# horizon-research/Fov-3DGS

Measured on AMD Instinct MI355X. Metric: frames/sec at 1080p foveated (bicycle-scale), higher is better.
Workload: dtype f32; 1 GPU; S-6M bicycle-scale cloud, 4-layer foveated render (fov_pcheck_obb), the reference's 9 fixed gazes (0.25 i, 0.25 j) in turn, one camera per GPU; gaussians=6000000, width=1920, height=1080, sh_degree=3, model_layout=the reference's tensor interface (render(packed=None)), overlap_successive_frames=True, parallelism=views1

## Files before the change

fov-3dgs_amd/csrc/api.hip:

```cpp
#include "common.h"
#include <atomic>
#include <mutex>
#include <cstdarg>
#include <cstdio>
#include <cstring>
#include <cstdlib>
#include <new>

namespace fr {

static thread_local char g_err[512] = "";

void set_error(const char *fmt, ...)
{
	va_list ap;
	va_start(ap, fmt);
	vsnprintf(g_err, sizeof(g_err), fmt, ap);
	va_end(ap);
}

int check_launch(const char *what, hipStream_t stream, bool debug)
{
	hipError_t e = hipGetLastError();
	static const bool trace = getenv("FR_TRACE") != nullptr;
// ... 3 lines not shown
	if (e != hipSuccess)
	{
		set_error("%s: %s", what, hipGetErrorString(e));
		return FR_ERR_HIP;
	}
	return FR_OK;
}

#define FR_HIP(call) do { hipError_t e_ = (call); if (e_ != hipSuccess) { set_error("%s: %s", #call, hipGetErrorString(e_)); return FR_ERR_HIP; } } while (0)

static int validate_forward(const fr_forward_args *a)
{
	if (!a) { set_error("null args"); return FR_ERR_INVALID; }
	if (a->variant < FR_VARIANT_ORIGINAL || a->variant > FR_VARIANT_MMFR_PCHECK_OBB) { set_error("unknown variant %d", a->variant); return FR_ERR_INVALID; }
	if (a->P < 0 || a->W <= 0 || a->H <= 0) { set_error("bad sizes P=%d W=%d H=%d", a->P, a->W, a->H); return FR_ERR_INVALID; }
	if (a->P > (1 << 30) || a->W > 16 * 65535 || a->H > 16 * 65535) { set_error("too large: P=%d (max 2^30) W=%d H=%d (max 65535 tiles per axis)", a->P, a->W, a->H); return FR_ERR_INVALID; }
	if ((int64_t)((a->W + FR_TILE - 1) / FR_TILE) * ((a->H + FR_TILE - 1) / FR_TILE) >= (1 << 29)) { set_error("too many tiles (W=%d H=%d)", a->W, a->H); return FR_ERR_INVALID; }
	if (!a->out_color) { set_error("out_color is null"); return FR_ERR_INVALID; }
	if (a->P == 0) return FR_OK;
	if (!a->means3D || !a->opacities || !a->viewmatrix || !a->projmatrix || !a->campos || !a->background || !a->radii)
	{ set_error("a required pointer is null"); return FR_ERR_INVALID; }
	if (!a->geometry_resize || !a->binning_resize || !a->image_resize) { set_error("resize callbacks are required"); return FR_ERR_INVALID; }
	const bool fov = a->variant == FR_VARIANT_FOV_PCHECK_OBB;
	if (fov)
	{
		if (a->shs_rest) { set_error("shs_rest is not used by the foveated variant (its shs already is the rest part)"); return FR_ERR_INVALID; }
		if (!a->shs || !a->shs_dcs || !a->highest_levels) { set_error("foveated variant needs shs (rest), shs_dcs and highest_levels"); return FR_ERR_INVALID; }
		if (a->M != 15) { set_error("foveated variant expects M=15 rest coefficients, got %d", a->M); return FR_ERR_INVALID; }
	}
	else if (a->variant == FR_VARIANT_NAIVE_FOV_PCHECK_OBB || a->variant == FR_VARIANT_MMFR_PCHECK_OBB)
	{
// ... 554 lines not shown
```

fov-3dgs_amd/csrc/common.h:

```cpp
#pragma once
#include <hip/hip_runtime.h>
#include <stdint.h>
#include <stddef.h>
#include "../../include/fovraster.h"

#define FR_TILE 16
#define FR_TILE_PIX 256
#define FR_FOV_LEVELS 4
#define FR_SORT_LDS_MAX 8192
#ifndef FR_BIN_THREADS
#define FR_BIN_THREADS 768
#endif
#define FR_BIN_BLOCKS 512
#define FR_PROJ_MAX_WAVES 8192
#define FR_CROW_PAD (64 * FR_PROJ_MAX_WAVES)
#define FR_LDS_HIST_MAX_TILES 16384
#define FR_ITEM_NONE 0xffffffffu
#define FR_LDS_HIST16_MAX_TILES 34816
#define FR_HIST16_MAX_SLABS (65535 / FR_BIN_THREADS)
#define FR_BIG_TNUM 64
#define FR_GIANT_TNUM 1024
#define FR_GIANT_MAX 64
#define FR_SORT_SPLIT_MIN 16384
#define FR_SORT_CHUNK_TARGET 960
// ... 12 lines not shown
__host__ __device__ inline size_t align_up(size_t x, size_t a = 256) { return (x + a - 1) / a * a; }

struct GeomWS {
	float4 *rec;
	float *cov3D;
	float4 *acc;
	float4 *wrec;
	float4 *lvl;
	uint32_t *lrange;
	uint32_t *slab_ctr;
	uint32_t *vis_list;
	uint32_t *vis_seg;
	uint32_t *proj_counts;
	uint32_t *wbase;
	float4 *crow;
	size_t bytes;
};
__host__ __device__ inline GeomWS carve_geom(int variant, size_t P, char *base)
{
	GeomWS g; size_t off = 0;
	g.rec = (float4 *)(base + off); off = align_up(off + P * 3 * sizeof(float4));
	const bool keeps = has_backward(variant);
	g.cov3D = (float *)(base + off); off = align_up(off + P * (keeps ? 16 : 6) * sizeof(float));
	g.acc = nullptr;
	if (keeps) { g.acc = (float4 *)(base + off); off = align_up(off + P * 4 * sizeof(float4)); }
	g.lvl = nullptr;
	g.wrec = (float4 *)(base + off); off = align_up(off + P * 4 * sizeof(float4));
	if (variant == FR_VARIANT_FOV_PCHECK_OBB) { g.lvl = (float4 *)(base + off); off = align_up(off + P * FR_FOV_LEVELS * sizeof(float4)); }
	g.lrange = (uint32_t *)(base + off); off = align_up(off + P * sizeof(uint32_t));
	g.slab_ctr = (uint32_t *)(base + off); off = align_up(off + FR_SLAB_CTR_WORDS * sizeof(uint32_t));
	g.vis_list = (uint32_t *)(base + off); off = align_up(off + P * sizeof(uint32_t));
	g.vis_seg = (uint32_t *)(base + off); off = align_up(off + (P + FR_CROW_PAD) * sizeof(uint32_t));
	g.proj_counts = (uint32_t *)(base + off); off = align_up(off + FR_PROJ_MAX_WAVES * sizeof(uint32_t));
	g.wbase = (uint32_t *)(base + off); off = align_up(off + (FR_PROJ_MAX_WAVES + 1) * sizeof(uint32_t));
	g.crow = nullptr;
	if (is_fov(variant)) { g.crow = (float4 *)(base + off); off = align_up(off + (P + FR_CROW_PAD) * 3 * sizeof(float4)); }
	g.bytes = off + 256;
	return g;
}

struct ImageWS {
	float *final_T;
	uint32_t *n_contrib;
	uint2 *ranges;
	uint32_t *tile_count;
	uint32_t *lv_bbox;
	uint32_t *totals;
	uint32_t *render_items;
	uint32_t *tile_order;
	float *tile_lv;
	uint32_t *hist;
// ... 299 lines not shown
```

fov-3dgs_amd/csrc/preprocess.hip:

```cpp
#include "common.h"
#include "tile_scan.h"
#include <cstdlib>

namespace fr {

struct M3 { float c[3][3]; };
__device__ __forceinline__ M3 m3_cols(float a0, float a1, float a2, float b0, float b1, float b2, float c0, float c1, float c2)
{
	M3 m; m.c[0][0] = a0; m.c[0][1] = a1; m.c[0][2] = a2; m.c[1][0] = b0; m.c[1][1] = b1; m.c[1][2] = b2;
	m.c[2][0] = c0; m.c[2][1] = c1; m.c[2][2] = c2; return m;
}
__device__ __forceinline__ M3 m3_mul(const M3 &a, const M3 &b)
{
	M3 r;
#pragma unroll
	for (int col = 0; col < 3; col++)
#pragma unroll
		for (int row = 0; row < 3; row++)
			r.c[col][row] = a.c[0][row] * b.c[col][0] + a.c[1][row] * b.c[col][1] + a.c[2][row] * b.c[col][2];
	return r;
}
__device__ __forceinline__ M3 m3_t(const M3 &a)
{
	M3 r;
// ... 996 lines not shown
			}
			else
			{
				gidx = (int)a.geom.vis_seg[slot];
				load_candidate<PACKED, FOV>(a, gidx, g);
			}
		}
		GeomOut go;
		geom_item<VARIANT>(a, cam_vm, cam_pm, s_lvbox, valid, gidx, g, !PACKED && !FOV && a.raw && a.cov3D_precomp == nullptr, go);
		if (valid)
		{
			a.radii[gidx] = go.alive ? go.radius : 0;
			if (a.visibility) a.visibility[gidx] = (go.alive && go.radius > 0) ? 1 : 0;
			a.geom.vis_list[item] = (uint32_t)gidx;
		}
		rows_store<4>(go.wrow, orec, a.geom.wrec + 4 * (size_t)slab * 64, nv, lane);
		rows_store<3>(go.rrow, orec, a.geom.rec + 3 * (size_t)slab * 64, nv, lane);
		if (a.write_cov3D)
		{
			rows_store<4>(go.stash, orec, (float4 *)a.geom.cov3D + 4 * (size_t)slab * 64, nv, lane);
			const float4 ac[4] = { make_float4(0.f, 0.f, 0.f, 0.f), make_float4(0.f, 0.f, 0.f, 0.f), make_float4(0.f, 0.f, 0.f, 0.f), make_float4(go.inv_qnorm, 0.f, 0.f, 0.f) };
			rows_store<4>(ac, orec, a.geom.acc + 4 * (size_t)slab * 64, nv, lane);
		}
#pragma unroll
		for (int i = 0; i < 4; i++) wr[i] = go.wrow[i];
		fpos = make_float3(go.rrow[1].z, go.rrow[1].w, go.rrow[2].x);
		fconic = make_float3(go.rrow[0].z, go.rrow[0].w, go.rrow[1].x);
	}
	const uint32_t idf = __float_as_uint(wr[2].x), xy = __float_as_uint(wr[2].z);
	const int idx = (int)(idf & 0x3fffffffu);
	const bool alive = item < V && ((idf >> 30) & 1u) != 0, boxtest = ((idf >> 31) & 1u) != 0;
	const float4 ev = make_float4(wr[0].z, wr[0].w, wr[1].x, wr[1].y);
	const float2 el = make_float2(wr[1].z, wr[1].w);
	const int x0 = (int)(xy & 0xffffu), y0 = (int)(xy >> 16), ow0 = (int)__float_as_uint(wr[2].w);
	const uint32_t tnum = alive ? __float_as_uint(wr[3].x) : 0u;
	const float hl = wr[3].y;
	uint32_t count = 0;
	float lowest = hl, highest = 0;
	bool be_blend = false;
	const bool in_place = alive && tnum == 1 && !boxtest;
	if (in_place)
	{
		bool keep = true;
		const int ti = y0 * a.gx + x0;
		if (FOV)
		{
			uint32_t lb;
			TILE_FILTER(ti, hl + 1, keep, lb);
			if (keep) { const float level = (float)(31 - __clz((int)(lb & 15u))); lowest = level; highest = level; be_blend = (lb & 16u) != 0u; }
		}
		if (keep) { BUMP_TILE(ti); count = 1; }
	}
	bool deferred = false;
	{
		uint32_t lvmask = 0;
		if (alive && !in_place && tnum >= FR_GIANT_TNUM)
		{
			const uint32_t slot = atomicAdd(&s_ng, 1u);
			if (slot < FR_GIANT_MAX) { s_gitem[slot] = item; deferred = true; }
		}
		const bool big = alive && !in_place && !deferred && tnum >= FR_BIG_TNUM;
		if (__ballot(big)) __builtin_amdgcn_s_setprio(3);
		for (unsigned long long bigm = __ballot(big); bigm; bigm &= bigm - 1)
		{
			const int L = __ffsll((long long)bigm) - 1;
			const int ox0 = bcast_i(x0, L), oy0 = bcast_i(y0, L), ow = bcast_i(ow0, L);
// ... 54 lines not shown
					const bool cx_ok = !((o2.y - tpx) < -8.0f || (o2.x - tpx) > 8.0f);
					const bool cy_ok = !((o2.w - tpy) < -8.0f || (o2.z - tpy) > 8.0f);
					const float xp = tpx + 8.0f - o0.x, xm = tpx - 8.0f - o0.x, yp = tpy + 8.0f - o0.y, ym = tpy - 8.0f - o0.y;
					const float a1p = xp * o0.z, a1m = xm * o0.z, b1p = yp * o0.w, b1m = ym * o0.w;
					const float mn1 = fminf(a1p, a1m) + fminf(b1p, b1m), mx1 = fmaxf(a1p, a1m) + fmaxf(b1p, b1m);
					const bool e1_ok = !(o1.z < mn1 || -o1.z > mx1);
					const float a2p = xp * o1.x, a2m = xm * o1.x, b2p = yp * o1.y, b2m = ym * o1.y;
					const float mn2 = fminf(a2p, a2m) + fminf(b2p, b2m), mx2 = fmaxf(a2p, a2m) + fmaxf(b2p, b2m);
					const bool e2_ok = !(o1.w < mn2 || -o1.w > mx2);
					pass = pass && cx_ok && cy_ok && e1_ok && e2_ok;
				}
				if (FOV) m = pass ? lb : 0u;
			}
			if (pass) BUMP_TILE(ti);
			const unsigned long long mine = seg_mask(seg_a, seg_b);
			count += (uint32_t)__popcll(__ballot(pass) & mine);
			if (FOV)
			{
#pragma unroll
				for (int bit = 0; bit < 5; bit++)
					if (__ballot((m >> bit) & 1u) & mine) lvmask |= 1u << bit;
			}
		}
		if (total != 0)
		{
			__builtin_amdgcn_fence(__ATOMIC_RELEASE, "wavefront");
			__builtin_amdgcn_wave_barrier();
		}
		if (FOV && (my_n != 0 || big) && count != 0) range_from_mask(lvmask, lowest, highest, be_blend);
	}
	const uint32_t lr = (alive && !deferred) ? range_word(count, lowest, highest, be_blend) : FR_ITEM_NONE;
	if (item < V && !deferred) a.geom.lrange[item] = lr;
	if (alive && !deferred && count == 0) { a.radii[idx] = 0; if (a.visibility) a.visibility[idx] = 0; }
	if (__any(lr != FR_ITEM_NONE))
	{
		float4 r[3], lv[FR_FOV_LEVELS];
		r[0] = make_float4(wr[0].x, wr[0].y, fconic.x, fconic.y);
		r[1] = make_float4(fconic.z, LEVELCOL ? hl : 0.0f, fpos.x, fpos.y);
		r[2] = make_float4(fpos.z, wr[2].y, (FOV && !LEVELCOL) ? hl : 0.0f, __int_as_float(idx));
#pragma unroll
		for (int l = 0; l < FR_FOV_LEVELS; l++) lv[l] = make_float4(0, 0, 0, 0);
		if (lr != FR_ITEM_NONE) colour_item<VARIANT, PACKED>(a, rows_ok, lr, r, lv);
		if (LEVELCOL) rows_store<4>(lv, orec, a.geom.lvl + 4 * (size_t)slab * 64, nv, lane);
		else rows_store<3>(r, orec, a.geom.rec + 3 * (size_t)slab * 64, nv, lane);
	}
	}
	__syncthreads();
// ... 11 lines not shown
	}
	__syncthreads();
	if ((int)threadIdx.x < ng)
	{
		const int gitem = s_gitem[threadIdx.x];
		const uint32_t gcount = s_gcount[threadIdx.x];
		const float4 w2 = a.geom.wrec[4 * (size_t)gitem + 2], w3 = a.geom.wrec[4 * (size_t)gitem + 3];
		float lowest = w3.y, highest = 0.0f;
		bool be_blend = false;
		if (FOV && gcount != 0) range_from_mask(s_gmask[threadIdx.x], lowest, highest, be_blend);
		const uint32_t lr = range_word(gcount, lowest, highest, be_blend);
		a.geom.lrange[gitem] = lr;
		if (gcount == 0)
		{
			const uint32_t gi = __float_as_uint(w2.x) & 0x3fffffffu;
			a.radii[gi] = 0;
			if (a.visibility) a.visibility[gi] = 0;
		}
		else
		{
			float4 r[3], lv[FR_FOV_LEVELS];
#pragma unroll
			for (int i = 0; i < 3; i++) r[i] = a.geom.rec[3 * (size_t)gitem + i];
#pragma unroll
			for (int l = 0; l < FR_FOV_LEVELS; l++) lv[l] = make_float4(0, 0, 0, 0);
			colour_item<VARIANT, PACKED>(a, rows_ok, lr, r, lv);
			if (LEVELCOL)
			{
#pragma unroll
				for (int l = 0; l < FR_FOV_LEVELS; l++) a.geom.lvl[(size_t)gitem * FR_FOV_LEVELS + l] = lv[l];
// ... 29 lines not shown
			tile_scan_body<FR_TILE_SCAN_THREADS, true>(a.ts, lds_hist);
		}
	}
}
#undef BUMP_TILE
#undef TILE_FILTER

struct EmitArgs {
	int P, gx, gy, T;
	const int *radii;
	GeomWS geom;
	const float *highest_levels;
	const float *tile_lv;
	const uint32_t *lv_bbox;
	int lds_tiles;
	const uint2 *ranges;
	uint32_t *cursor;
	uint64_t *entries;
	const uint32_t *hist;
	const uint32_t *totals;
	uint32_t capacity;
	uint32_t items_cap;
};
#ifndef FR_EMIT_THREADS
#define FR_EMIT_THREADS FR_BIN_THREADS
#endif
#define NEXT_SLOT(ti) (LDSH == 2 ? a.ranges[(ti)].x + pre_row[(ti)] + ((atomicAdd(&lds_cur[(ti) >> 1], 1u << (16 * ((ti) & 1))) >> (16 * ((ti) & 1))) & 0xffffu) \
	: LDSH ? atomicAdd(&lds_cur[(ti)], 1u) : a.ranges[(ti)].x + atomicAdd(&a.cursor[(ti)], 1u))
template <int VARIANT, int LDSH>
__global__ void __launch_bounds__(FR_EMIT_THREADS) k_emit(const EmitArgs a)
{
	constexpr bool CULL = VARIANT != FR_VARIANT_ORIGINAL;
	constexpr bool FOV = VARIANT == FR_VARIANT_FOV_PCHECK_OBB;
	extern __shared__ __attribute__((aligned(16))) uint32_t lds_cur[];
#ifdef FR_EMIT_TIMERS
	const uint64_t tm_entry = wall_clock64(); uint64_t tm_pro = 0, tm_loop = 0, tm_walk = 0, tm_big = 0, tm_drain = 0, tm_pre = 0, tm_mid = 0, tm_ta = 0; int tm_slabs = 0, tm_steps = 0;
#endif
	if (a.totals[0] > a.capacity || a.totals[5] > a.items_cap) return;
	const int lane = threadIdx.x & 63;
	const int cur_words = LDSH == 2 ? (a.T + 1) / 2 : (LDSH ? a.T : 0);
	const uint32_t *const pre_row = a.hist + (LDSH ? (size_t)blockIdx.x * a.T : 0);
	uint32_t *lds_tab = lds_cur + cur_words;
	const int tab_words = (a.T + 7) / 8;
	const bool ldst = FOV && a.lds_tiles && a.geom.slab_ctr[3] == 0u;
	if (ldst)
	{
		const float *gmin = a.tile_lv + a.T;
		for (int t0 = threadIdx.x; t0 < a.T; t0 += 16 * FR_EMIT_THREADS)
		{
			float v[16];
#pragma unroll
// ... 12 lines not shown
#define TILE_PASSES(ti, olim) (ldst ? (float)((lds_tab[(ti) >> 3] >> (4 * ((ti) & 7))) & 7u) < (olim) : tile_min[(ti)] < (olim))
	if (LDSH == 2)
		for (int t = threadIdx.x; t < cur_words; t += FR_EMIT_THREADS) lds_cur[t] = 0;
	else if (LDSH)
	{
		const uint32_t *pre = pre_row;
		for (int t0 = threadIdx.x; t0 < a.T; t0 += 16 * FR_EMIT_THREADS)
		{
			uint32_t st[16], pr[16];
#pragma unroll
			for (int k = 0; k < 16; k++) { const int t = min(t0 + k * FR_EMIT_THREADS, a.T - 1); st[k] = a.ranges[t].x; pr[k] = pre[t]; }
#pragma unroll
			for (int k = 0; k < 16; k++) if (t0 + k * FR_EMIT_THREADS < a.T) lds_cur[t0 + k * FR_EMIT_THREADS] = st[k] + pr[k];
		}
	}
	__syncthreads();
	__shared__ int s_own[FR_EMIT_THREADS];
	float4 *const s_orec = (float4 *)(lds_cur + ((cur_words + (ldst ? tab_words : 0) + 3) & ~3));
	__shared__ int s_gidx[FR_GIANT_MAX];
	__shared__ uint32_t s_ng, s_next_slab;
	if (threadIdx.x == 0) { s_ng = 0; s_next_slab = 0; }
	__syncthreads();
#ifdef FR_EMIT_TIMERS
	tm_pro = wall_clock64() - tm_entry;
#endif
	const float *tile_min = FOV ? a.tile_lv + a.T : nullptr;
	auto walk_uniform = [&](const int ox0, const int oy0, const int ow, const uint32_t on, const Obb &ob, const float olim,
		const uint64_t opay, const uint32_t k0, const uint32_t kstep) __attribute__((always_inline))
	{
		const float rw = 1.0f / (float)ow;
		for (uint32_t k = k0; k < on; k += kstep)
		{
			const uint32_t j = k + lane;
			const bool valid = j < on;
			int ry = (int)(((float)j + 0.5f) * rw);
			int rx = (int)j - ry * ow;
			if (rx < 0) { ry--; rx += ow; } else if (rx >= ow) { ry++; rx -= ow; }
			const int x = ox0 + rx, y = oy0 + ry;
			const int ti = valid ? y * a.gx + x : 0;
			bool pass = valid;
			if (CULL)
			{
				if (FOV) pass = pass && TILE_PASSES(ti, olim);
				pass = pass && obb_hits_tile(ob, x, y);
			}
			if (pass) a.entries[NEXT_SLOT(ti)] = opay;
		}
	};
	const int V = (int)a.geom.slab_ctr[1];
	const int nslabs = (V + 63) / 64;
	struct SlabIn { float4 w0, w1, w2, w3; uint32_t lr; };
	auto fetch_slab = [&](const int slab, SlabIn &in) __attribute__((always_inline))
	{
		const int item = min(slab * 64 + lane, max(V - 1, 0));
		const float4 *wr = a.geom.wrec + 4 * (size_t)item;
		in.lr = a.geom.lrange[item];
		in.w0 = wr[0]; in.w1 = wr[1]; in.w2 = wr[2]; in.w3 = wr[3];
	};
	auto process = [&](const int slab, const SlabIn &in) __attribute__((always_inline))
	{
	const int item = slab * 64 + lane;
	int idx = 0;
	bool alive = false, boxtest = false;
	int x0 = 0, y0 = 0, x1 = 0;
	uint32_t tnum = 0;
	float cx = 0.f, cy = 0.f, hl = 0.f;
	uint32_t depth_bits = 0;
	float4 ev = make_float4(0, 0, 0, 0);
	float2 el = make_float2(0, 0);
	if (item < V)
	{
		const uint32_t lr = in.lr;
		const float4 w0 = in.w0, w1 = in.w1, w2 = in.w2, w3 = in.w3;
		const uint32_t idf = __float_as_uint(w2.x), xy = __float_as_uint(w2.z);
		idx = (int)(idf & 0x3fffffffu);
		alive = lr != FR_ITEM_NONE && ((idf >> 30) & 1u) != 0; boxtest = (idf >> 31) & 1u;
		cx = w0.x; cy = w0.y; ev = make_float4(w0.z, w0.w, w1.x, w1.y); el = make_float2(w1.z, w1.w);
		depth_bits = __float_as_uint(w2.y);
		x0 = (int)(xy & 0xffffu); y0 = (int)(xy >> 16); x1 = x0 + (int)__float_as_uint(w2.w);
		tnum = alive ? __float_as_uint(w3.x) : 0u;
		hl = w3.y;
	}
	const uint64_t payload = ((uint64_t)depth_bits << 32) | (uint32_t)item;
	const bool in_place = alive && tnum == 1 && !boxtest;
	if (in_place) a.entries[NEXT_SLOT(y0 * a.gx + x0)] = payload;
	{
		bool deferred = false;
		if (alive && !in_place && tnum >= FR_GIANT_TNUM)
		{
			const uint32_t slot = atomicAdd(&s_ng, 1u);
			if (slot < FR_GIANT_MAX) { s_gidx[slot] = item; deferred = true; }
		}
		const bool big = alive && !in_place && !deferred && tnum >= FR_BIG_TNUM;
#ifdef FR_EMIT_TIMERS
		const uint64_t tg0 = wall_clock64(); tm_pre += tg0 - tm_ta;
#endif
		for (unsigned long long bigm = __ballot(big); bigm; bigm &= bigm - 1)
		{
			const int L = __ffsll((long long)bigm) - 1;
			const int ox0 = bcast_i(x0, L), oy0 = bcast_i(y0, L), ow = bcast_i(x1, L) - ox0;
			const float4 oev = make_float4(bcast_f(ev.x, L), bcast_f(ev.y, L), bcast_f(ev.z, L), bcast_f(ev.w, L));
			const float2 oel = make_float2(bcast_f(el.x, L), bcast_f(el.y, L));
			const Obb ob = make_obb(bcast_f(cx, L), bcast_f(cy, L), oev, oel);
			const uint64_t opay = ((uint64_t)(uint32_t)bcast_i((int)depth_bits, L) << 32) | (uint32_t)(slab * 64 + L);
			walk_uniform(ox0, oy0, ow, (uint32_t)bcast_i((int)tnum, L), ob, bcast_f(hl, L) + 1, opay, 0u, 64u);
		}
#ifdef FR_EMIT_TIMERS
		const uint64_t tg1 = wall_clock64(); tm_big += tg1 - tg0;
#endif
		const uint32_t my_n = (alive && !in_place && !big && !deferred) ? tnum : 0u;
		const uint32_t incl = wave_incl_scan_u32(my_n, lane);
		const uint32_t excl = incl - my_n;
		const uint32_t total = (uint32_t)__builtin_amdgcn_readlane((int)incl, 63);
		float4 *const orec = s_orec + 4 * (threadIdx.x & ~63);
#ifdef FR_EMIT_TIMERS
		const uint64_t tw0 = wall_clock64(); tm_steps += (int)((total + 63) / 64); tm_mid += tw0 - tg1;
#endif
		if (total != 0)
		{
			const Obb ob = make_obb(cx, cy, ev, el);
			float4 *mine = orec + 4 * lane;
			mine[0] = make_float4(cx, cy, ev.x, ev.y);
			mine[1] = make_float4(ev.z, ev.w, el.x, el.y);
			mine[2] = make_float4(ob.vxmin, ob.vxmax, ob.vymin, ob.vymax);
			mine[3] = make_float4(__uint_as_float((uint32_t)x0 | ((uint32_t)y0 << 16)), __int_as_float(max(x1 - x0, 1)), __uint_as_float(excl), hl + 1);
			FR_WAVE_LDS_SYNC();
		}
		for (uint32_t k = 0; k < total; k += 64)
		{
			const uint32_t j = k + lane;
			const bool valid = j < total;
			const int seg_a = (int)max((long long)excl - (long long)k, 0ll);
			const int seg_b = (int)min((long long)incl - (long long)k, 64ll);
			const int owner = max(pair_owner_scan(s_own + (threadIdx.x & ~63), lane, seg_a, seg_b), 0);
			const float4 *orow = orec + 4 * owner;
			const float4 o3 = orow[3];
			const uint32_t oxy = __float_as_uint(o3.x);
			const int ow = __float_as_int(o3.y);
			const uint32_t local = (valid ? j : total - 1) - __float_as_uint(o3.z);
			int qy = (int)(((float)local + 0.5f) * __builtin_amdgcn_rcpf((float)ow));
			int rx = (int)local - qy * ow;
			if (rx < 0) { qy--; rx += ow; } else if (rx >= ow) { qy++; rx -= ow; }
			const int x = (int)(oxy & 0xffffu) + rx, y = (int)(oxy >> 16) + qy;
			const int ti = y * a.gx + x;
			const uint64_t opay = ((uint64_t)(uint32_t)__shfl((int)depth_bits, owner) << 32) | (uint32_t)(slab * 64 + owner);
			bool pass = valid;
			if (CULL)
			{
				const float4 o0 = orow[0], o1 = orow[1], o2 = orow[2];
				if (FOV) pass = pass && TILE_PASSES(valid ? ti : 0, o3.w);
				{
					const float tpx = (float)x * (float)FR_TILE + (float)FR_TILE / 2.0f, tpy = (float)y * (float)FR_TILE + (float)FR_TILE / 2.0f;
					const bool cx_ok = !((o2.y - tpx) < -8.0f || (o2.x - tpx) > 8.0f);
					const bool cy_ok = !((o2.w - tpy) < -8.0f || (o2.z - tpy) > 8.0f);
					const float xp = tpx + 8.0f - o0.x, xm = tpx - 8.0f - o0.x, yp = tpy + 8.0f - o0.y, ym = tpy - 8.0f - o0.y;
					const float a1p = xp * o0.z, a1m = xm * o0.z, b1p = yp * o0.w, b1m = ym * o0.w;
					const float mn1 = fminf(a1p, a1m) + fminf(b1p, b1m), mx1 = fmaxf(a1p, a1m) + fmaxf(b1p, b1m);
					const bool e1_ok = !(o1.z < mn1 || -o1.z > mx1);
					const float a2p = xp * o1.x, a2m = xm * o1.x, b2p = yp * o1.y, b2m = ym * o1.y;
					const float mn2 = fminf(a2p, a2m) + fminf(b2p, b2m), mx2 = fmaxf(a2p, a2m) + fmaxf(b2p, b2m);
					const bool e2_ok = !(o1.w < mn2 || -o1.w > mx2);
					pass = pass && cx_ok && cy_ok && e1_ok && e2_ok;
				}
			}
			if (pass) a.entries[NEXT_SLOT(ti)] = opay;
		}
		if (total != 0)
		{
			__builtin_amdgcn_fence(__ATOMIC_RELEASE, "wavefront");
			__builtin_amdgcn_wave_barrier();
		}
#ifdef FR_EMIT_TIMERS
		tm_walk += wall_clock64() - tw0;
#endif
	}
	};
	{
		constexpr int BW = FR_BIN_THREADS / 64;
		const int bin_waves = (int)gridDim.x * BW;
		auto slab_of = [&](const int s) { return (int)blockIdx.x * BW + s % BW + (s / BW) * bin_waves; };
		auto grab = [&]() -> int {
			uint32_t q_ = 0;
			if (lane == 0) q_ = atomicAdd(&s_next_slab, 1u);
			return slab_of(__builtin_amdgcn_readfirstlane((int)q_));
		};
		SlabIn cur, nxt;
		int slab = grab();
		if (slab < nslabs) fetch_slab(slab, cur);
#ifdef FR_EMIT_TIMERS
		const uint64_t tl0 = wall_clock64();
#endif
		for (; slab < nslabs; )
		{
#ifdef FR_EMIT_TIMERS
			tm_ta = wall_clock64();
#endif
			const int next = grab();
			const bool more = next < nslabs;
			if (more) fetch_slab(next, nxt);
			process(slab, cur);
#ifdef FR_EMIT_TIMERS
			{ const uint64_t td0 = wall_clock64(); asm volatile("s_waitcnt vmcnt(0)" ::: "memory"); tm_drain += wall_clock64() - td0; }
#endif
			if (more) cur = nxt;
			slab = next;
#ifdef FR_EMIT_TIMERS
			tm_slabs++;
#endif
		}
#ifdef FR_EMIT_TIMERS
		tm_loop = wall_clock64() - tl0;
#endif
	}
#ifdef FR_EMIT_TIMERS
	const uint64_t tb0 = wall_clock64();
#endif
	__syncthreads();
#ifdef FR_EMIT_TIMERS
	if (lane == 0)
	{
		float *d = a.geom.cov3D + (size_t)((int)blockIdx.x * (FR_EMIT_THREADS / 64) + (int)(threadIdx.x >> 6)) * 8;
		d[0] = (float)(wall_clock64() - tm_entry); d[1] = (float)tm_pro; d[2] = (float)tm_loop; d[3] = (float)(wall_clock64() - tb0);
		d[4] = (float)tm_slabs; d[5] = (float)tm_steps; d[6] = (float)tm_walk; d[7] = (float)tm_big; d[3] = (float)tm_drain; d[1] = (float)tm_pre; d[4] = (float)tm_mid;
	}
#endif
	const int ng = min((int)s_ng, FR_GIANT_MAX);
	for (int g = 0; g < ng; g++)
	{
		const float4 *wr = a.geom.wrec + 4 * (size_t)s_gidx[g];
		const float4 w0 = wr[0], w1 = wr[1], w2 = wr[2], w3 = wr[3];
		const Obb ob = make_obb(w0.x, w0.y, make_float4(w0.z, w0.w, w1.x, w1.y), make_float2(w1.z, w1.w));
		const uint32_t xy = __float_as_uint(w2.z);
		const uint64_t opay = ((uint64_t)__float_as_uint(w2.y) << 32) | (uint32_t)s_gidx[g];
		walk_uniform((int)(xy & 0xffffu), (int)(xy >> 16), (int)__float_as_uint(w2.w), __float_as_uint(w3.x), ob, w3.y + 1, opay,
			(uint32_t)(threadIdx.x & ~63u), (uint32_t)FR_EMIT_THREADS);
	}
}
#undef NEXT_SLOT
#undef TILE_PASSES

__global__ void k_mark_visible(int P, const float *means3D, const float *vm, uint8_t *present)
{
	const int idx = blockIdx.x * blockDim.x + threadIdx.x;
	if (idx >= P) return;
	const float z = vm[2] * means3D[3 * idx] + vm[6] * means3D[3 * idx + 1] + vm[10] * means3D[3 * idx + 2] + vm[14];
	present[idx] = !(z <= 0.2f);
}

__global__ void k_pack_geom(int P, const float *means3D, const float *scales, const float *rotations, const float *opacities,
	int levels, const float *highest_levels, float4 *out)
// ... 207 lines not shown
	c.bin_wgs = nblk;
	return check_launch("bin", c.stream, a->debug);
}

int launch_emit(FwdCtx &c)
{
	const fr_forward_args *a = c.a;
	EmitArgs e;
	e.P = a->P; e.gx = c.gx; e.gy = c.gy; e.T = c.T; e.radii = a->radii; e.geom = c.geom;
	e.highest_levels = a->highest_levels; e.tile_lv = c.img.tile_lv; e.lv_bbox = c.img.lv_bbox; e.ranges = c.img.ranges;
	e.cursor = c.img.tile_count; e.entries = c.bin.entries; e.hist = c.img.hist;
	e.totals = c.img.totals; e.capacity = (uint32_t)c.capacity; e.items_cap = (uint32_t)c.items_cap;
	const bool ldsh = c.hist_mode != 0;
	const dim3 grid(c.bin_wgs), block(FR_EMIT_THREADS);
	e.lds_tiles = (is_fov(a->variant) && ldsh) ? 1 : 0;
	const size_t lds = (((c.hist_mode == 2 ? (size_t)((c.T + 1) / 2) * sizeof(uint32_t) : (ldsh ? (size_t)c.T * sizeof(uint32_t) : 0)) +
		(e.lds_tiles ? lds_tile_table_bytes(c.T) : 0) + 15) & ~(size_t)15) + (size_t)FR_EMIT_THREADS * 4 * sizeof(float4);
	if (lds > 64u * 1024u)
	{
		static const hipError_t once = []() {
			const void *fns[] = { (const void *)k_emit<FR_VARIANT_ORIGINAL, 0>, (const void *)k_emit<FR_VARIANT_ORIGINAL, 1>, (const void *)k_emit<FR_VARIANT_ORIGINAL, 2>,
				(const void *)k_emit<FR_VARIANT_PCHECK_OBB, 0>, (const void *)k_emit<FR_VARIANT_PCHECK_OBB, 1>, (const void *)k_emit<FR_VARIANT_PCHECK_OBB, 2>,
				(const void *)k_emit<FR_VARIANT_FOV_PCHECK_OBB, 0>, (const void *)k_emit<FR_VARIANT_FOV_PCHECK_OBB, 1>, (const void *)k_emit<FR_VARIANT_FOV_PCHECK_OBB, 2> };
			for (const void *fn : fns)
			{
				const hipError_t e1 = hipFuncSetAttribute(fn, hipFuncAttributeMaxDynamicSharedMemorySize, (FR_EMIT_THREADS > 768 ? 154 : 156) * 1024);
				if (e1 != hipSuccess) return e1;
			}
			return hipSuccess; }();
		if (once != hipSuccess) { set_error("hipFuncSetAttribute(k_emit): %s", hipGetErrorString(once)); return FR_ERR_HIP; }
	}
#define LAUNCH_EMIT(V) do { if (c.hist_mode == 2) hipLaunchKernelGGL((k_emit<V, 2>), grid, block, lds, c.stream, e); \
	else if (ldsh) hipLaunchKernelGGL((k_emit<V, 1>), grid, block, lds, c.stream, e); \
	else hipLaunchKernelGGL((k_emit<V, 0>), grid, block, lds, c.stream, e); } while (0)
	switch (a->variant)
	{
	case FR_VARIANT_ORIGINAL: LAUNCH_EMIT(FR_VARIANT_ORIGINAL); break;
	case FR_VARIANT_FOV_PCHECK_OBB:
	case FR_VARIANT_MMFR_PCHECK_OBB:
	case FR_VARIANT_NAIVE_FOV_PCHECK_OBB: LAUNCH_EMIT(FR_VARIANT_FOV_PCHECK_OBB); break;
	default: LAUNCH_EMIT(FR_VARIANT_PCHECK_OBB); break;
// ... 13 lines not shown
```

Measured before the change: 2176 frames/s.

## Emit from compact per-item tile-mask records staged in LDS rounds

The bin pass now records, for each visible item, a 64-bit mask of the tiles that passed culling plus packed origin, width, depth and a kind tag (none, masked, big, giant). Emit loads these compact records in rounds into LDS and scatters entries by selecting the n-th set bit, so it no longer reruns the OBB and foveation tile test or reads the full 64-byte wrec rows for small items. wrec is written only for waves that contain big items, and big or giant rows are staged in LDS. The cost is an extra 16-byte per-item record, a tighter LDS budget, a new cap of 4096 tiles per axis, and a block-level sync per round in place of the previous prefetch pipeline.

```diff
diff --git a/fov-3dgs_amd/csrc/api.hip b/fov-3dgs_amd/csrc/api.hip
--- a/fov-3dgs_amd/csrc/api.hip
+++ b/fov-3dgs_amd/csrc/api.hip
@@ -41,7 +41,7 @@
 	if (!a) { set_error("null args"); return FR_ERR_INVALID; }
 	if (a->variant < FR_VARIANT_ORIGINAL || a->variant > FR_VARIANT_MMFR_PCHECK_OBB) { set_error("unknown variant %d", a->variant); return FR_ERR_INVALID; }
 	if (a->P < 0 || a->W <= 0 || a->H <= 0) { set_error("bad sizes P=%d W=%d H=%d", a->P, a->W, a->H); return FR_ERR_INVALID; }
-	if (a->P > (1 << 30) || a->W > 16 * 65535 || a->H > 16 * 65535) { set_error("too large: P=%d (max 2^30) W=%d H=%d (max 65535 tiles per axis)", a->P, a->W, a->H); return FR_ERR_INVALID; }
+	if (a->P > (1 << 30) || a->W > 16 * FR_EREC_MAX_GRID || a->H > 16 * FR_EREC_MAX_GRID) { set_error("too large: P=%d (max 2^30) W=%d H=%d (max %d tiles per axis)", a->P, a->W, a->H, FR_EREC_MAX_GRID); return FR_ERR_INVALID; }
 	if ((int64_t)((a->W + FR_TILE - 1) / FR_TILE) * ((a->H + FR_TILE - 1) / FR_TILE) >= (1 << 29)) { set_error("too many tiles (W=%d H=%d)", a->W, a->H); return FR_ERR_INVALID; }
 	if (!a->out_color) { set_error("out_color is null"); return FR_ERR_INVALID; }
 	if (a->P == 0) return FR_OK;
diff --git a/fov-3dgs_amd/csrc/common.h b/fov-3dgs_amd/csrc/common.h
--- a/fov-3dgs_amd/csrc/common.h
+++ b/fov-3dgs_amd/csrc/common.h
@@ -50,8 +50,18 @@
 	uint32_t *proj_counts;
 	uint32_t *wbase;
 	float4 *crow;
+	uint4 *erec;
 	size_t bytes;
 };
+#define FR_EREC_NONE 0u
+#define FR_EREC_MASKED 1u
+#define FR_EREC_BIG 2u
+#define FR_EREC_GIANT 3u
+#define FR_EREC_MAX_GRID 4096
+__host__ __device__ inline uint32_t erec_word(int x0, int y0, int width, uint32_t kind)
+{
+	return (uint32_t)(x0 & 0xfff) | ((uint32_t)(y0 & 0xfff) << 12) | ((uint32_t)((width - 1) & 63) << 24) | (kind << 30);
+}
 __host__ __device__ inline GeomWS carve_geom(int variant, size_t P, char *base)
 {
 	GeomWS g; size_t off = 0;
@@ -71,6 +81,7 @@
 	g.wbase = (uint32_t *)(base + off); off = align_up(off + (FR_PROJ_MAX_WAVES + 1) * sizeof(uint32_t));
 	g.crow = nullptr;
 	if (is_fov(variant)) { g.crow = (float4 *)(base + off); off = align_up(off + (P + FR_CROW_PAD) * 3 * sizeof(float4)); }
+	g.erec = (uint4 *)(base + off); off = align_up(off + P * sizeof(uint4));
 	g.bytes = off + 256;
 	return g;
 }
diff --git a/fov-3dgs_amd/csrc/preprocess.hip b/fov-3dgs_amd/csrc/preprocess.hip
--- a/fov-3dgs_amd/csrc/preprocess.hip
+++ b/fov-3dgs_amd/csrc/preprocess.hip
@@ -1034,7 +1034,12 @@
 			if (a.visibility) a.visibility[gidx] = (go.alive && go.radius > 0) ? 1 : 0;
 			a.geom.vis_list[item] = (uint32_t)gidx;
 		}
-		rows_store<4>(go.wrow, orec, a.geom.wrec + 4 * (size_t)slab * 64, nv, lane);
+#ifdef FR_WREC_ALL
+		const bool keep_wrec = true;
+#else
+		const bool keep_wrec = __any(__float_as_uint(go.wrow[3].x) >= FR_BIG_TNUM);
+#endif
+		if (keep_wrec) rows_store<4>(go.wrow, orec, a.geom.wrec + 4 * (size_t)slab * 64, nv, lane);
 		rows_store<3>(go.rrow, orec, a.geom.rec + 3 * (size_t)slab * 64, nv, lane);
 		if (a.write_cov3D)
 		{
@@ -1056,6 +1061,7 @@
 	const uint32_t tnum = alive ? __float_as_uint(wr[3].x) : 0u;
 	const float hl = wr[3].y;
 	uint32_t count = 0;
+	unsigned long long tmask = 0;
 	float lowest = hl, highest = 0;
 	bool be_blend = false;
 	const bool in_place = alive && tnum == 1 && !boxtest;
@@ -1069,7 +1075,7 @@
 			TILE_FILTER(ti, hl + 1, keep, lb);
 			if (keep) { const float level = (float)(31 - __clz((int)(lb & 15u))); lowest = level; highest = level; be_blend = (lb & 16u) != 0u; }
 		}
-		if (keep) { BUMP_TILE(ti); count = 1; }
+		if (keep) { BUMP_TILE(ti); count = 1; tmask = 1ull; }
 	}
 	bool deferred = false;
 	{
@@ -1154,7 +1160,9 @@
 			}
 			if (pass) BUMP_TILE(ti);
 			const unsigned long long mine = seg_mask(seg_a, seg_b);
-			count += (uint32_t)__popcll(__ballot(pass) & mine);
+			const unsigned long long kept = __ballot(pass) & mine;
+			count += (uint32_t)__popcll(kept);
+			if (seg_b > seg_a) tmask |= (kept >> seg_a) << (k + (uint32_t)seg_a - excl);
 			if (FOV)
 			{
 #pragma unroll
@@ -1171,6 +1179,11 @@
 	}
 	const uint32_t lr = (alive && !deferred) ? range_word(count, lowest, highest, be_blend) : FR_ITEM_NONE;
 	if (item < V && !deferred) a.geom.lrange[item] = lr;
+	if (item < V)
+	{
+		const uint32_t kind = deferred ? FR_EREC_GIANT : (lr == FR_ITEM_NONE ? FR_EREC_NONE : (tnum >= FR_BIG_TNUM ? FR_EREC_BIG : FR_EREC_MASKED));
+		a.geom.erec[item] = make_uint4((uint32_t)tmask, (uint32_t)(tmask >> 32), __float_as_uint(wr[2].y), erec_word(x0, y0, max(ow0, 1), kind));
+	}
 	if (alive && !deferred && count == 0) { a.radii[idx] = 0; if (a.visibility) a.visibility[idx] = 0; }
 	if (__any(lr != FR_ITEM_NONE))
 	{
@@ -1212,6 +1225,7 @@
 		if (gcount == 0)
 		{
 			const uint32_t gi = __float_as_uint(w2.x) & 0x3fffffffu;
+			a.geom.erec[gitem].w = 0u;
 			a.radii[gi] = 0;
 			if (a.visibility) a.visibility[gi] = 0;
 		}
@@ -1271,6 +1285,7 @@
 	const float *tile_lv;
 	const uint32_t *lv_bbox;
 	int lds_tiles;
+	int round_slabs;
 	const uint2 *ranges;
 	uint32_t *cursor;
 	uint64_t *entries;
@@ -1282,6 +1297,24 @@
 #ifndef FR_EMIT_THREADS
 #define FR_EMIT_THREADS FR_BIN_THREADS
 #endif
+#ifndef FR_EMIT_PLAIN
+#define FR_EMIT_PLAIN 0
+#endif
+#define FR_EMIT_WBIG 128
+__device__ __forceinline__ uint32_t nth_set_bit(const unsigned long long m, uint32_t n)
+{
+	const uint32_t lo = (uint32_t)m, hi = (uint32_t)(m >> 32);
+	uint32_t c = (uint32_t)__popc(lo), base = 0;
+	uint32_t w = lo;
+	if (n >= c) { n -= c; w = hi; base = 32; }
+#pragma unroll
+	for (int h = 16; h >= 2; h >>= 1)
+	{
+		c = (uint32_t)__popc(w & ((1u << h) - 1u));
+		if (n >= c) { n -= c; w >>= h; base += (uint32_t)h; }
+	}
+	return base + (n >= (w & 1u) ? 1u : 0u);
+}
 #define NEXT_SLOT(ti) (LDSH == 2 ? a.ranges[(ti)].x + pre_row[(ti)] + ((atomicAdd(&lds_cur[(ti) >> 1], 1u << (16 * ((ti) & 1))) >> (16 * ((ti) & 1))) & 0xffffu) \
 	: LDSH ? atomicAdd(&lds_cur[(ti)], 1u) : a.ranges[(ti)].x + atomicAdd(&a.cursor[(ti)], 1u))
 template <int VARIANT, int LDSH>
@@ -1291,7 +1324,7 @@
 	constexpr bool FOV = VARIANT == FR_VARIANT_FOV_PCHECK_OBB;
 	extern __shared__ __attribute__((aligned(16))) uint32_t lds_cur[];
 #ifdef FR_EMIT_TIMERS
-	const uint64_t tm_entry = wall_clock64(); uint64_t tm_pro = 0, tm_loop = 0, tm_walk = 0, tm_big = 0, tm_drain = 0, tm_pre = 0, tm_mid = 0, tm_ta = 0; int tm_slabs = 0, tm_steps = 0;
+	const uint64_t tm_entry = wall_clock64(); uint64_t tm_pro = 0, tm_walk = 0, tm_big = 0, tm_round = 0; int tm_slabs = 0, tm_steps = 0;
 #endif
 	if (a.totals[0] > a.capacity || a.totals[5] > a.items_cap) return;
 	const int lane = threadIdx.x & 63;
@@ -1334,17 +1367,16 @@
 			for (int k = 0; k < 16; k++) if (t0 + k * FR_EMIT_THREADS < a.T) lds_cur[t0 + k * FR_EMIT_THREADS] = st[k] + pr[k];
 		}
 	}
-	__syncthreads();
 	__shared__ int s_own[FR_EMIT_THREADS];
-	float4 *const s_orec = (float4 *)(lds_cur + ((cur_words + (ldst ? tab_words : 0) + 3) & ~3));
+	uint4 *const s_rec = (uint4 *)(lds_cur + ((cur_words + (ldst ? tab_words : 0) + 3) & ~3));
+	float4 *const s_wbig = (float4 *)(s_rec + (size_t)max(a.round_slabs, 1) * 64);
 	__shared__ int s_gidx[FR_GIANT_MAX];
-	__shared__ uint32_t s_ng, s_next_slab;
-	if (threadIdx.x == 0) { s_ng = 0; s_next_slab = 0; }
-	__syncthreads();
-#ifdef FR_EMIT_TIMERS
-	tm_pro = wall_clock64() - tm_entry;
-#endif
+	__shared__ uint32_t s_ng, s_next_slab, s_nbig;
+	__shared__ float4 s_grow[4 * FR_GIANT_MAX];
+	__shared__ int s_gstaged[FR_GIANT_MAX];
+	if (threadIdx.x == 0) s_ng = 0;
 	const float *tile_min = FOV ? a.tile_lv + a.T : nullptr;
+	const float4 *__restrict__ const wrec = a.geom.wrec;
 	auto walk_uniform = [&](const int ox0, const int oy0, const int ow, const uint32_t on, const Obb &ob, const float olim,
 		const uint64_t opay, const uint32_t k0, const uint32_t kstep) __attribute__((always_inline))
 	{
@@ -1367,85 +1399,63 @@
 			if (pass) a.entries[NEXT_SLOT(ti)] = opay;
 		}
 	};
+	auto walk_item = [&](const float4 w0, const float4 w1, const float4 w2, const float4 w3, const int witem, const uint32_t k0, const uint32_t kstep) __attribute__((always_inline))
+	{
+		const Obb ob = make_obb(w0.x, w0.y, make_float4(w0.z, w0.w, w1.x, w1.y), make_float2(w1.z, w1.w));
+		const uint32_t xy = __float_as_uint(w2.z);
+		const uint64_t opay = ((uint64_t)__float_as_uint(w2.y) << 32) | (uint32_t)witem;
+		walk_uniform((int)(xy & 0xffffu), (int)(xy >> 16), (int)__float_as_uint(w2.w), __float_as_uint(w3.x), ob, w3.y + 1, opay, k0, kstep);
+	};
 	const int V = (int)a.geom.slab_ctr[1];
 	const int nslabs = (V + 63) / 64;
-	struct SlabIn { float4 w0, w1, w2, w3; uint32_t lr; };
-	auto fetch_slab = [&](const int slab, SlabIn &in) __attribute__((always_inline))
-	{
-		const int item = min(slab * 64 + lane, max(V - 1, 0));
-		const float4 *wr = a.geom.wrec + 4 * (size_t)item;
-		in.lr = a.geom.lrange[item];
-		in.w0 = wr[0]; in.w1 = wr[1]; in.w2 = wr[2]; in.w3 = wr[3];
-	};
-	auto process = [&](const int slab, const SlabIn &in) __attribute__((always_inline))
-	{
-	const int item = slab * 64 + lane;
-	int idx = 0;
-	bool alive = false, boxtest = false;
-	int x0 = 0, y0 = 0, x1 = 0;
-	uint32_t tnum = 0;
-	float cx = 0.f, cy = 0.f, hl = 0.f;
-	uint32_t depth_bits = 0;
-	float4 ev = make_float4(0, 0, 0, 0);
-	float2 el = make_float2(0, 0);
-	if (item < V)
-	{
-		const uint32_t lr = in.lr;
-		const float4 w0 = in.w0, w1 = in.w1, w2 = in.w2, w3 = in.w3;
-		const uint32_t idf = __float_as_uint(w2.x), xy = __float_as_uint(w2.z);
-		idx = (int)(idf & 0x3fffffffu);
-		alive = lr != FR_ITEM_NONE && ((idf >> 30) & 1u) != 0; boxtest = (idf >> 31) & 1u;
-		cx = w0.x; cy = w0.y; ev = make_float4(w0.z, w0.w, w1.x, w1.y); el = make_float2(w1.z, w1.w);
-		depth_bits = __float_as_uint(w2.y);
-		x0 = (int)(xy & 0xffffu); y0 = (int)(xy >> 16); x1 = x0 + (int)__float_as_uint(w2.w);
-		tnum = alive ? __float_as_uint(w3.x) : 0u;
-		hl = w3.y;
-	}
-	const uint64_t payload = ((uint64_t)depth_bits << 32) | (uint32_t)item;
-	const bool in_place = alive && tnum == 1 && !boxtest;
-	if (in_place) a.entries[NEXT_SLOT(y0 * a.gx + x0)] = payload;
-	{
-		bool deferred = false;
-		if (alive && !in_place && tnum >= FR_GIANT_TNUM)
+	constexpr int BW = FR_BIN_THREADS / 64;
+	const int bin_waves = (int)gridDim.x * BW;
+	auto slab_of = [&](const int s) { return (int)blockIdx.x * BW + s % BW + (s / BW) * bin_waves; };
+	const int nshare = (nslabs / bin_waves) * BW + min(max(nslabs % bin_waves - (int)blockIdx.x * BW, 0), BW);
+	const int R = max(a.round_slabs, 1);
+	auto process = [&](const int s, const int rs) __attribute__((always_inline))
+	{
+		const int slab = slab_of(s);
+		const uint4 *const rrow = s_rec + (size_t)(s - rs) * 64;
+		const uint4 rec = rrow[lane];
+		const uint32_t kind = rec.w >> 30;
+		if (kind == FR_EREC_GIANT)
 		{
 			const uint32_t slot = atomicAdd(&s_ng, 1u);
-			if (slot < FR_GIANT_MAX) { s_gidx[slot] = item; deferred = true; }
-		}
-		const bool big = alive && !in_place && !deferred && tnum >= FR_BIG_TNUM;
+			if (slot < FR_GIANT_MAX)
+			{
+				s_gidx[slot] = slab * 64 + lane;
+				const bool staged = rec.x < FR_EMIT_WBIG;
+				s_gstaged[slot] = staged ? 1 : 0;
+				if (staged)
+				{
+#pragma unroll
+					for (int i = 0; i < 4; i++) s_grow[4 * slot + i] = s_wbig[4 * rec.x + i];
+				}
+			}
+		}
 #ifdef FR_EMIT_TIMERS
-		const uint64_t tg0 = wall_clock64(); tm_pre += tg0 - tm_ta;
+		const uint64_t tg0 = wall_clock64();
 #endif
-		for (unsigned long long bigm = __ballot(big); bigm; bigm &= bigm - 1)
+		for (unsigned long long bigm = __ballot(kind == FR_EREC_BIG); bigm; bigm &= bigm - 1)
 		{
 			const int L = __ffsll((long long)bigm) - 1;
-			const int ox0 = bcast_i(x0, L), oy0 = bcast_i(y0, L), ow = bcast_i(x1, L) - ox0;
-			const float4 oev = make_float4(bcast_f(ev.x, L), bcast_f(ev.y, L), bcast_f(ev.z, L), bcast_f(ev.w, L));
-			const float2 oel = make_float2(bcast_f(el.x, L), bcast_f(el.y, L));
-			const Obb ob = make_obb(bcast_f(cx, L), bcast_f(cy, L), oev, oel);
-			const uint64_t opay = ((uint64_t)(uint32_t)bcast_i((int)depth_bits, L) << 32) | (uint32_t)(slab * 64 + L);
-			walk_uniform(ox0, oy0, ow, (uint32_t)bcast_i((int)tnum, L), ob, bcast_f(hl, L) + 1, opay, 0u, 64u);
+			const uint32_t bslot = (uint32_t)__builtin_amdgcn_readlane((int)rec.x, L);
+			const int witem = slab * 64 + L;
+			if (bslot < FR_EMIT_WBIG) { const float4 *wr = s_wbig + 4 * bslot; walk_item(wr[0], wr[1], wr[2], wr[3], witem, 0u, 64u); }
+			else { const float4 *wr = wrec + 4 * (size_t)witem; walk_item(wr[0], wr[1], wr[2], wr[3], witem, 0u, 64u); }
 		}
 #ifdef FR_EMIT_TIMERS
-		const uint64_t tg1 = wall_clock64(); tm_big += tg1 - tg0;
+		const uint64_t tw0 = wall_clock64(); tm_big += tw0 - tg0;
 #endif
-		const uint32_t my_n = (alive && !in_place && !big && !deferred) ? tnum : 0u;
+		const unsigned long long mask = kind == FR_EREC_MASKED ? (((unsigned long long)rec.y << 32) | rec.x) : 0ull;
+		const uint32_t my_n = FR_EMIT_PLAIN ? (mask ? 64u - (uint32_t)__clzll((long long)mask) : 0u) : (uint32_t)__popcll(mask);
 		const uint32_t incl = wave_incl_scan_u32(my_n, lane);
 		const uint32_t excl = incl - my_n;
 		const uint32_t total = (uint32_t)__builtin_amdgcn_readlane((int)incl, 63);
-		float4 *const orec = s_orec + 4 * (threadIdx.x & ~63);
 #ifdef FR_EMIT_TIMERS
-		const uint64_t tw0 = wall_clock64(); tm_steps += (int)((total + 63) / 64); tm_mid += tw0 - tg1;
+		tm_steps += (int)((total + 63) / 64);
 #endif
-		if (total != 0)
-		{
-			const Obb ob = make_obb(cx, cy, ev, el);
-			float4 *mine = orec + 4 * lane;
-			mine[0] = make_float4(cx, cy, ev.x, ev.y);
-			mine[1] = make_float4(ev.z, ev.w, el.x, el.y);
-			mine[2] = make_float4(ob.vxmin, ob.vxmax, ob.vymin, ob.vymax);
-			mine[3] = make_float4(__uint_as_float((uint32_t)x0 | ((uint32_t)y0 << 16)), __int_as_float(max(x1 - x0, 1)), __uint_as_float(excl), hl + 1);
-			FR_WAVE_LDS_SYNC();
-		}
 		for (uint32_t k = 0; k < total; k += 64)
 		{
 			const uint32_t j = k + lane;
@@ -1453,84 +1463,75 @@
 			const int seg_a = (int)max((long long)excl - (long long)k, 0ll);
 			const int seg_b = (int)min((long long)incl - (long long)k, 64ll);
 			const int owner = max(pair_owner_scan(s_own + (threadIdx.x & ~63), lane, seg_a, seg_b), 0);
-			const float4 *orow = orec + 4 * owner;
-			const float4 o3 = orow[3];
-			const uint32_t oxy = __float_as_uint(o3.x);
-			const int ow = __float_as_int(o3.y);
-			const uint32_t local = (valid ? j : total - 1) - __float_as_uint(o3.z);
+			const uint4 o = rrow[owner];
+			const uint32_t n = (valid ? j : total - 1) - (uint32_t)__shfl((int)excl, owner);
+			const unsigned long long omask = ((unsigned long long)o.y << 32) | o.x;
+			const uint32_t local = FR_EMIT_PLAIN ? n : nth_set_bit(omask, n);
+			const bool pass = valid && (!FR_EMIT_PLAIN || ((omask >> local) & 1ull) != 0ull);
+			const int ow = (int)((o.w >> 24) & 63u) + 1;
 			int qy = (int)(((float)local + 0.5f) * __builtin_amdgcn_rcpf((float)ow));
 			int rx = (int)local - qy * ow;
 			if (rx < 0) { qy--; rx += ow; } else if (rx >= ow) { qy++; rx -= ow; }
-			const int x = (int)(oxy & 0xffffu) + rx, y = (int)(oxy >> 16) + qy;
-			const int ti = y * a.gx + x;
-			const uint64_t opay = ((uint64_t)(uint32_t)__shfl((int)depth_bits, owner) << 32) | (uint32_t)(slab * 64 + owner);
-			bool pass = valid;
-			if (CULL)
-			{
-				const float4 o0 = orow[0], o1 = orow[1], o2 = orow[2];
-				if (FOV) pass = pass && TILE_PASSES(valid ? ti : 0, o3.w);
+			const int ti = ((int)((o.w >> 12) & 0xfffu) + qy) * a.gx + (int)(o.w & 0xfffu) + rx;
+			if (pass) a.entries[NEXT_SLOT(ti)] = ((uint64_t)o.z << 32) | (uint32_t)(slab * 64 + owner);
+		}
+#ifdef FR_EMIT_TIMERS
+		tm_walk += wall_clock64() - tw0; tm_slabs++;
+#endif
+	};
+	for (int rs = 0; rs < nshare; rs += R)
+	{
+#ifdef FR_EMIT_TIMERS
+		const uint64_t tr0 = wall_clock64();
+#endif
+		const int rn = min(R, nshare - rs), ne = rn * 64;
+		if (threadIdx.x == 0) s_nbig = 0;
+		__syncthreads();
+		for (int e0 = threadIdx.x; e0 < ne; e0 += 16 * FR_EMIT_THREADS)
+		{
+			uint4 v[16];
+#pragma unroll
+			for (int k = 0; k < 16; k++)
+			{
+				const int e = min(e0 + k * FR_EMIT_THREADS, ne - 1);
+				v[k] = a.geom.erec[min(slab_of(rs + (e >> 6)) * 64 + (e & 63), V - 1)];
+			}
+#pragma unroll
+			for (int k = 0; k < 16; k++)
+			{
+				const int e = e0 + k * FR_EMIT_THREADS;
+				if (e < ne)
 				{
-					const float tpx = (float)x * (float)FR_TILE + (float)FR_TILE / 2.0f, tpy = (float)y * (float)FR_TILE + (float)FR_TILE / 2.0f;
-					const bool cx_ok = !((o2.y - tpx) < -8.0f || (o2.x - tpx) > 8.0f);
-					const bool cy_ok = !((o2.w - tpy) < -8.0f || (o2.z - tpy) > 8.0f);
-					const float xp = tpx + 8.0f - o0.x, xm = tpx - 8.0f - o0.x, yp = tpy + 8.0f - o0.y, ym = tpy - 8.0f - o0.y;
-					const float a1p = xp * o0.z, a1m = xm * o0.z, b1p = yp * o0.w, b1m = ym * o0.w;
-					const float mn1 = fminf(a1p, a1m) + fminf(b1p, b1m), mx1 = fmaxf(a1p, a1m) + fmaxf(b1p, b1m);
-					const bool e1_ok = !(o1.z < mn1 || -o1.z > mx1);
-					const float a2p = xp * o1.x, a2m = xm * o1.x, b2p = yp * o1.y, b2m = ym * o1.y;
-					const float mn2 = fminf(a2p, a2m) + fminf(b2p, b2m), mx2 = fmaxf(a2p, a2m) + fmaxf(b2p, b2m);
-					const bool e2_ok = !(o1.w < mn2 || -o1.w > mx2);
-					pass = pass && cx_ok && cy_ok && e1_ok && e2_ok;
+					const int item = slab_of(rs + (e >> 6)) * 64 + (e & 63);
+					const uint32_t w = item >= V ? 0u : v[k].w;
+					uint32_t x = v[k].x;
+					if ((w >> 30) >= FR_EREC_BIG)
+					{
+						x = atomicAdd(&s_nbig, 1u);
+						if (x < FR_EMIT_WBIG)
+						{
+							const float4 *wr = wrec + 4 * (size_t)item;
+							const float4 w0 = wr[0], w1 = wr[1], w2 = wr[2], w3 = wr[3];
+							s_wbig[4 * x] = w0; s_wbig[4 * x + 1] = w1; s_wbig[4 * x + 2] = w2; s_wbig[4 * x + 3] = w3;
+						}
+					}
+					s_rec[e] = make_uint4(x, v[k].y, v[k].z, w);
 				}
 			}
-			if (pass) a.entries[NEXT_SLOT(ti)] = opay;
-		}
-		if (total != 0)
-		{
-			__builtin_amdgcn_fence(__ATOMIC_RELEASE, "wavefront");
-			__builtin_amdgcn_wave_barrier();
-		}
+		}
+		if (threadIdx.x == 0) s_next_slab = (uint32_t)rs;
+		__syncthreads();
 #ifdef FR_EMIT_TIMERS
-		tm_walk += wall_clock64() - tw0;
+		if (rs == 0) tm_pro = wall_clock64() - tm_entry; else tm_round += wall_clock64() - tr0;
 #endif
-	}
-	};
-	{
-		constexpr int BW = FR_BIN_THREADS / 64;
-		const int bin_waves = (int)gridDim.x * BW;
-		auto slab_of = [&](const int s) { return (int)blockIdx.x * BW + s % BW + (s / BW) * bin_waves; };
-		auto grab = [&]() -> int {
+		for (;;)
+		{
 			uint32_t q_ = 0;
 			if (lane == 0) q_ = atomicAdd(&s_next_slab, 1u);
-			return slab_of(__builtin_amdgcn_readfirstlane((int)q_));
-		};
-		SlabIn cur, nxt;
-		int slab = grab();
-		if (slab < nslabs) fetch_slab(slab, cur);
-#ifdef FR_EMIT_TIMERS
-		const uint64_t tl0 = wall_clock64();
-#endif
-		for (; slab < nslabs; )
-		{
-#ifdef FR_EMIT_TIMERS
-			tm_ta = wall_clock64();
-#endif
-			const int next = grab();
-			const bool more = next < nslabs;
-			if (more) fetch_slab(next, nxt);
-			process(slab, cur);
-#ifdef FR_EMIT_TIMERS
-			{ const uint64_t td0 = wall_clock64(); asm volatile("s_waitcnt vmcnt(0)" ::: "memory"); tm_drain += wall_clock64() - td0; }
-#endif
-			if (more) cur = nxt;
-			slab = next;
-#ifdef FR_EMIT_TIMERS
-			tm_slabs++;
-#endif
-		}
-#ifdef FR_EMIT_TIMERS
-		tm_loop = wall_clock64() - tl0;
-#endif
+			const int s = __builtin_amdgcn_readfirstlane((int)q_);
+			if (s >= rs + rn) break;
+			process(s, rs);
+		}
 	}
 #ifdef FR_EMIT_TIMERS
 	const uint64_t tb0 = wall_clock64();
@@ -1540,20 +1541,16 @@
 	if (lane == 0)
 	{
 		float *d = a.geom.cov3D + (size_t)((int)blockIdx.x * (FR_EMIT_THREADS / 64) + (int)(threadIdx.x >> 6)) * 8;
-		d[0] = (float)(wall_clock64() - tm_entry); d[1] = (float)tm_pro; d[2] = (float)tm_loop; d[3] = (float)(wall_clock64() - tb0);
-		d[4] = (float)tm_slabs; d[5] = (float)tm_steps; d[6] = (float)tm_walk; d[7] = (float)tm_big; d[3] = (float)tm_drain; d[1] = (float)tm_pre; d[4] = (float)tm_mid;
+		d[0] = (float)(wall_clock64() - tm_entry); d[1] = (float)tm_pro; d[2] = (float)tm_round; d[3] = (float)(wall_clock64() - tb0);
+		d[4] = (float)tm_slabs; d[5] = (float)tm_steps; d[6] = (float)tm_walk; d[7] = (float)tm_big;
 	}
 #endif
 	const int ng = min((int)s_ng, FR_GIANT_MAX);
 	for (int g = 0; g < ng; g++)
 	{
-		const float4 *wr = a.geom.wrec + 4 * (size_t)s_gidx[g];
-		const float4 w0 = wr[0], w1 = wr[1], w2 = wr[2], w3 = wr[3];
-		const Obb ob = make_obb(w0.x, w0.y, make_float4(w0.z, w0.w, w1.x, w1.y), make_float2(w1.z, w1.w));
-		const uint32_t xy = __float_as_uint(w2.z);
-		const uint64_t opay = ((uint64_t)__float_as_uint(w2.y) << 32) | (uint32_t)s_gidx[g];
-		walk_uniform((int)(xy & 0xffffu), (int)(xy >> 16), (int)__float_as_uint(w2.w), __float_as_uint(w3.x), ob, w3.y + 1, opay,
-			(uint32_t)(threadIdx.x & ~63u), (uint32_t)FR_EMIT_THREADS);
+		const int witem = s_gidx[g];
+		if (s_gstaged[g]) { const float4 *wr = s_grow + 4 * g; walk_item(wr[0], wr[1], wr[2], wr[3], witem, (uint32_t)(threadIdx.x & ~63u), (uint32_t)FR_EMIT_THREADS); }
+		else { const float4 *wr = wrec + 4 * (size_t)witem; walk_item(wr[0], wr[1], wr[2], wr[3], witem, (uint32_t)(threadIdx.x & ~63u), (uint32_t)FR_EMIT_THREADS); }
 	}
 }
 #undef NEXT_SLOT
@@ -1791,8 +1788,21 @@
 	const bool ldsh = c.hist_mode != 0;
 	const dim3 grid(c.bin_wgs), block(FR_EMIT_THREADS);
 	e.lds_tiles = (is_fov(a->variant) && ldsh) ? 1 : 0;
-	const size_t lds = (((c.hist_mode == 2 ? (size_t)((c.T + 1) / 2) * sizeof(uint32_t) : (ldsh ? (size_t)c.T * sizeof(uint32_t) : 0)) +
-		(e.lds_tiles ? lds_tile_table_bytes(c.T) : 0) + 15) & ~(size_t)15) + (size_t)FR_EMIT_THREADS * 4 * sizeof(float4);
+	if (c.gx > FR_EREC_MAX_GRID || c.gy > FR_EREC_MAX_GRID) { set_error("tile grid %d x %d exceeds %d tiles per axis", c.gx, c.gy, FR_EREC_MAX_GRID); return FR_ERR_INVALID; }
+	const size_t lds_fixed = ((c.hist_mode == 2 ? (size_t)((c.T + 1) / 2) * sizeof(uint32_t) : (ldsh ? (size_t)c.T * sizeof(uint32_t) : 0)) +
+		(e.lds_tiles ? lds_tile_table_bytes(c.T) : 0) + 15) & ~(size_t)15;
+	const size_t lds_wbig = (size_t)FR_EMIT_WBIG * 4 * sizeof(float4);
+	const size_t lds_cap = (size_t)(FR_EMIT_THREADS > 768 ? 148 : 150) * 1024 - lds_wbig;
+	static const int round_env = []() { const char *s = getenv("FOVRASTER_EMIT_ROUND_SLABS"); const int v = s ? atoi(s) : 0; return v > 0 ? v : 0; }();
+	const int64_t bin_waves = (int64_t)c.bin_wgs * (FR_BIN_THREADS / 64);
+	const int64_t cand_slabs = ((int64_t)(a->num_candidates > 0 ? a->num_candidates : 0) + 63) / 64;
+	const int64_t share = (cand_slabs + bin_waves - 1) / bin_waves * (FR_BIN_THREADS / 64);
+	int64_t round_slabs = (int64_t)((lds_cap - lds_fixed) / (64 * sizeof(uint4)));
+	if (round_slabs > share) round_slabs = share;
+	if (round_env > 0 && round_slabs > round_env) round_slabs = round_env;
+	if (round_slabs < 1) round_slabs = 1;
+	e.round_slabs = (int)round_slabs;
+	const size_t lds = lds_fixed + (size_t)round_slabs * 64 * sizeof(uint4) + lds_wbig;
 	if (lds > 64u * 1024u)
 	{
 		static const hipError_t once = []() {
@@ -1801,7 +1811,7 @@
 				(const void *)k_emit<FR_VARIANT_FOV_PCHECK_OBB, 0>, (const void *)k_emit<FR_VARIANT_FOV_PCHECK_OBB, 1>, (const void *)k_emit<FR_VARIANT_FOV_PCHECK_OBB, 2> };
 			for (const void *fn : fns)
 			{
-				const hipError_t e1 = hipFuncSetAttribute(fn, hipFuncAttributeMaxDynamicSharedMemorySize, (FR_EMIT_THREADS > 768 ? 154 : 156) * 1024);
+				const hipError_t e1 = hipFuncSetAttribute(fn, hipFuncAttributeMaxDynamicSharedMemorySize, (FR_EMIT_THREADS > 768 ? 148 : 150) * 1024);
 				if (e1 != hipSuccess) return e1;
 			}
 			return hipSuccess; }();
```

New measurement: 2210 frames/s (median of 2 runs). About the same (+1.6%).
